# vsahni3/cross-attention-ViT

Hardware: AMD Instinct MI355X
Metric: 3D patch-tokens/sec fwd+bwd, 2-modality 128^3 p16 ViT (higher is better)
Workload: dtype bf16; 1 GPU; configs[1]: ModelCross d=768 H=12 mlp=3072 2x2 blocks, 2 modalities, 128^3 volume, 16^3 patches (N=513), dropout 0; per_gpu_batch=126, global_batch=126, seq_len=513, parallelism=dp1, step=zero-grad + weight bf16 cast + fwd + loss + bwd, optimizer_step=excluded, launch=eager (one launch per kernel)

## Files before the change

cross-attention-vit_amd/csrc/gemm.hip:

```cpp
#include "xvit_common.h"

#include <atomic>
#include <algorithm>
#include <string>

namespace xvit {

struct GemmParams {
  const bf16* A = nullptr; const bf16* B = nullptr; void* C = nullptr; const float* bias = nullptr; const float* res = nullptr; bf16* aux = nullptr;
  int64_t lda = 0, ldb = 0, ldc = 0, ldr = 0, ldaux = 0;
  int64_t sA = 0, sB = 0, sC = 0, sBias = 0, sR = 0, sAux = 0;
  int M = 0, N = 0, K = 0, k_per_split = 0, split_k = 1, ntm = 0, ntn = 0;
  int c_f32 = 0, act = XVIT_ACT_NONE, accumulate = 0;
  int res_row_mod = 0, res_row_off = 0, seg_rows = 0, seg_skip = 0, row_off = 0;
  float* slab = nullptr;
  float* colsum = nullptr;
  float drop_p = 0.f, drop_inv = 1.f; uint64_t drop_seed = 0;
  const uint64_t* drop_epoch = nullptr;
  int aux_deriv = 0;
  int narrow_epi = 0;
  int ncg = 1;
  int res_in_body = 0;
  struct PatchGather {
    int mode = 0;
// ... 508 lines not shown
template <int ACT, bool DROP, int R, bool PERM = false, bool RESPF = false>
__device__ __forceinline__ void big_epi_regions(const GemmParams& p, BigEpi& e, LoadCursor& lc, EpiLoads& cur, const f32x4 (&acc)[8][4], XVIT_LDS char* slice,
                                                const uint32_t (&woff)[8], const uint32_t (&roff)[4]) {
  if constexpr ((R & 3) == 0) {
#pragma unroll
    for (int i = 0; i < 4; ++i)
#pragma unroll
      for (int j = 0; j < 4; ++j) {
        if constexpr (PERM) *(XVIT_LDS f32x4*)(slice + (i >> 1) * 8192 + woff[(i & 1) * 4 + j]) = acc[(R >> 2) * 4 + i][j];
        else *(XVIT_LDS f32x4*)(slice + i * 4096 + woff[j]) = acc[(R >> 2) * 4 + i][j];
      }
  }
  EpiLoads nxt;
  if constexpr (ACT == XVIT_ACT_DGELU && R < 7) big_epi_issue_aux(p, e, lc, nxt);
  if constexpr (RESPF && R < 7) big_epi_issue_res(p, e, lc, nxt);
#pragma unroll
  for (int b = 0; b < 4; ++b) {
    const int it = (R & 3) * 4 + b;
    const f32x4 v = *(const XVIT_LDS f32x4*)(slice + it * 1024 + roff[it & 3]);
    big_epi_body<ACT, DROP, RESPF>(p, e, v, cur.aux[b], cur.res[b]);
  }
  __builtin_amdgcn_sched_barrier(0);
  if constexpr (R < 7) big_epi_regions<ACT, DROP, R + 1, PERM, RESPF>(p, e, lc, nxt, acc, slice, woff, roff);
}

template <int ACT, bool DROP, bool PERM = false, bool RESPF = false>
__device__ __forceinline__ void big_epilogue(const GemmParams& p, BigEpi& e, const f32x4 (&acc)[8][4], XVIT_LDS char* slice, const uint32_t (&woff)[8],
                                             const uint32_t (&roff)[4]) {
  LoadCursor lc = {e.row, e.aux, e.res, e.rrem};
  EpiLoads first;
  if constexpr (ACT == XVIT_ACT_DGELU) big_epi_issue_aux(p, e, lc, first);
  if constexpr (RESPF) big_epi_issue_res(p, e, lc, first);
  big_epi_regions<ACT, DROP, 0, PERM, RESPF>(p, e, lc, first, acc, slice, woff, roff);
  if (p.colsum && !e.to_slab) colsum_flush<16>(e.colsum_dst, e.csum, e.col_ok);
}

__device__ __forceinline__ int pin_lane(int lane) {
  int pin = 0;
  asm volatile("" : "+v"(pin));
  return lane + pin;
}

struct Transpose8 {
  uint32_t woff[4], roffw[2][2];
  __device__ __forceinline__ void init(int wl) {
    const int r = wl & 15, g = wl >> 4, c = wl & 7, rr = wl >> 3;
#pragma unroll
    for (int j = 0; j < 4; ++j) woff[j] = (uint32_t)(r * 256 + (((j * 4 + g) ^ r) << 4));
#pragma unroll
    for (int par = 0; par < 2; ++par)
#pragma unroll
      for (int k = 0; k < 2; ++k) roffw[par][k] = (uint32_t)(rr * 256 + (((2 * c + k) ^ ((par * 8 + rr) & 15)) << 4));
  }
  template <int PASS>
  __device__ __forceinline__ void write(XVIT_LDS char* slice, const f32x4 (&acc)[8][4]) const {
#pragma unroll
    for (int i = 0; i < 4; ++i)
#pragma unroll
      for (int j = 0; j < 4; ++j) *(XVIT_LDS f32x4*)(slice + i * 4096 + woff[j]) = acc[PASS * 4 + i][j];
  }
  __device__ __forceinline__ void read(const XVIT_LDS char* slice, int it, f32x4& v0, f32x4& v1) const {
    v0 = *(const XVIT_LDS f32x4*)(slice + it * 2048 + roffw[it & 1][0]);
    v1 = *(const XVIT_LDS f32x4*)(slice + it * 2048 + roffw[it & 1][1]);
  }
};
template <int R, class Loads, class Prefetch, class Body>
__device__ __forceinline__ void transpose8_regions(const Transpose8& t, const f32x4 (&acc)[8][4], XVIT_LDS char* slice, Loads& cur, const Prefetch& prefetch, const Body& body) {
  if constexpr ((R & 3) == 0) t.write<(R >> 2)>(slice, acc);
  Loads nxt;
  if constexpr (R < 7) prefetch(nxt);
#pragma unroll
  for (int b = 0; b < 2; ++b) {
    f32x4 v0, v1;
    t.read(slice, (R & 3) * 2 + b, v0, v1);
    body(v0, v1, cur, b);
  }
  __builtin_amdgcn_sched_barrier(0);
  if constexpr (R < 7) transpose8_regions<R + 1>(t, acc, slice, nxt, prefetch, body);
}

typedef __attribute__((ext_vector_type(8))) float f32x8;
struct WideEpi {
  __amdgpu_buffer_rsrc_t rc, raux;
  bool has_aux, col_ok;
  uint32_t col;
  f32x4 bias0, bias1, csum0, csum1;
  uint64_t drop_base;
  uint32_t row, c, aux, c_step, aux_step;
};
struct WideCursor { uint32_t row, aux; };
struct WideLoads { u32x4_t aux[2]; };

__device__ __forceinline__ void wide_issue_aux(const GemmParams& p, const WideEpi& e, WideCursor& lc, WideLoads& L) {
#pragma unroll
  for (int b = 0; b < 2; ++b) {
    const bool ok = e.col_ok && lc.row < (uint32_t)p.M;
    L.aux[b] = __builtin_amdgcn_raw_buffer_load_b128(e.raux, ok ? lc.aux : OOB, 0, XVIT_EPI_LOAD_AUX);
    lc.row += 8; lc.aux += e.aux_step;
  }
}

__device__ __forceinline__ u32x4_t pack_bf16x8(const f32x4& a, const f32x4& b) {
  return __builtin_bit_cast(u32x4_t, to_bf16x8(a, b));
}

template <int ACT, bool DROP>
__device__ __forceinline__ void wide_half(const GemmParams& p, f32x4& v, const bf16x4 z, uint64_t idx, u32x2_t& dpack) {
  f32x4 d;
  act4<ACT>(v, d, z);
  if (ACT == ACT_GELU_D) {
    dpack = __builtin_bit_cast(u32x2_t, to_bf16x4(d));
  }
  if (DROP) dropout4(p, v, idx);
}

template <int ACT, bool DROP>
__device__ __forceinline__ void wide_body(const GemmParams& p, WideEpi& e, f32x4 v0, f32x4 v1, u32x4_t auxv) {
  const bool ok = e.col_ok && e.row < (uint32_t)p.M;
  v0 += e.bias0; v1 += e.bias1;
  if (ACT == XVIT_ACT_GELU && e.has_aux) __builtin_amdgcn_raw_buffer_store_b128(pack_bf16x8(v0, v1), e.raux, ok ? e.aux : OOB, 0, XVIT_EPI_STORE_AUX);
  const bf16x8 z = __builtin_bit_cast(bf16x8, auxv);
  const uint64_t idx = e.drop_base + (uint64_t)e.row * p.N + e.col;
  u32x2_t d0 = {0u, 0u}, d1 = {0u, 0u};
  wide_half<ACT, DROP>(p, v0, bf16x4{z[0], z[1], z[2], z[3]}, idx, d0);
  if ((ACT != XVIT_ACT_NONE && ACT != ACT_MULAUX) || DROP) __builtin_amdgcn_sched_barrier(0);
  wide_half<ACT, DROP>(p, v1, bf16x4{z[4], z[5], z[6], z[7]}, idx + 4, d1);
  if (ACT == ACT_GELU_D && e.has_aux) __builtin_amdgcn_raw_buffer_store_b128(u32x4_t{d0[0], d0[1], d1[0], d1[1]}, e.raux, ok ? e.aux : OOB, 0, XVIT_EPI_STORE_AUX);
  __builtin_amdgcn_raw_buffer_store_b128(pack_bf16x8(v0, v1), e.rc, ok ? e.c : OOB, 0, XVIT_EPI_STORE_AUX);
#pragma unroll
  for (int c = 0; c < 4; ++c) { e.csum0[c] += ok ? v0[c] : 0.f; e.csum1[c] += ok ? v1[c] : 0.f; }
  e.row += 8; e.c += e.c_step; e.aux += e.aux_step;
}

template <int ACT, bool DROP>
__device__ __forceinline__ void wide_epilogue(const GemmParams& p, WideEpi& e, const f32x4 (&acc)[8][4], XVIT_LDS char* slice, const Transpose8& t, float* colsum_dst) {
  WideCursor lc = {e.row, e.aux};
  const auto prefetch = [&](WideLoads& L) {
    if constexpr (ACT == XVIT_ACT_DGELU || ACT == ACT_MULAUX) wide_issue_aux(p, e, lc, L);
  };
  WideLoads first;
  prefetch(first);
  transpose8_regions<0>(t, acc, slice, first, prefetch, [&](f32x4 v0, f32x4 v1, const WideLoads& cur, int b) { wide_body<ACT, DROP>(p, e, v0, v1, cur.aux[b]); });
  if (colsum_dst) {
    colsum_flush<8>(colsum_dst, e.csum0, e.col_ok);
    colsum_flush<8>(colsum_dst + 4, e.csum1, e.col_ok);
  }
}

template <int ACT>
__device__ __forceinline__ void wave_tile_epilogue_wide(const GemmParams& p, const f32x4 (&acc)[8][4], XVIT_LDS char* smem, int wave, int lane, int row0, int col0,
                                                        int batch) {
  WideEpi e;
  e.rc = make_rsrc((const char*)p.C + batch * p.sC * 2, clamp_bytes(0x7FFFFFF0ll));
  e.has_aux = p.aux != nullptr;
  const bool has_bias = p.bias != nullptr;
  e.raux = make_rsrc(e.has_aux ? (const void*)(p.aux + batch * p.sAux) : (const void*)p.C, e.has_aux ? 0x7FFFFFF0u : 0u);
  const __amdgpu_buffer_rsrc_t rbias = make_rsrc(has_bias ? (const void*)(p.bias + batch * p.sBias) : (const void*)p.C, has_bias ? (uint32_t)(p.N * 4) : 0u);
  const int wl = pin_lane(lane);
  Transpose8 t;
  t.init(wl);
  XVIT_LDS char* slice = smem + wave * EPI_WAVE_BYTES;
  e.col = (uint32_t)(col0 + (wl & 7) * 8);
  e.col_ok = e.col < (uint32_t)p.N;
  e.bias0 = __builtin_bit_cast(f32x4, __builtin_amdgcn_raw_buffer_load_b128(rbias, e.col * 4, 0, 0));
  e.bias1 = __builtin_bit_cast(f32x4, __builtin_amdgcn_raw_buffer_load_b128(rbias, e.col * 4 + 16, 0, 0));
  e.drop_base = (uint64_t)batch * ((uint64_t)p.M * p.N);
  e.csum0 = f32x4{0.f, 0.f, 0.f, 0.f}; e.csum1 = f32x4{0.f, 0.f, 0.f, 0.f};
  float* colsum_dst = p.colsum ? p.colsum + batch * p.sBias + e.col : nullptr;
  e.row = (uint32_t)(row0 + (wl >> 3));
  e.c = e.row * (uint32_t)p.ldc * 2u + e.col * 2u;
  e.aux = e.row * (uint32_t)p.ldaux * 2u + e.col * 2u;
  e.c_step = 8u * (uint32_t)p.ldc * 2u;
  e.aux_step = 8u * (uint32_t)p.ldaux * 2u;
  wide_epilogue<ACT, false>(p, e, acc, slice, t, colsum_dst);
}

template <bool PERM = false, bool RES_PF = true>
__device__ __forceinline__ void wave_tile_epilogue(const GemmParams& p, const f32x4 (&acc)[8][4], XVIT_LDS char* smem, int wave, int lane, int row0, int col0,
                                                   int batch, int split) {
  const int nbatch = gridDim.z / p.split_k;
  BigEpi e;
  const int64_t celt = p.c_f32 ? 4 : 2;
  e.rc = make_rsrc((const char*)p.C + batch * p.sC * celt, clamp_bytes(0x7FFFFFF0ll));
  e.has_aux = p.aux != nullptr; e.has_res = p.res != nullptr; e.to_slab = p.slab != nullptr;
  const bool has_bias = p.bias != nullptr;
  e.raux = make_rsrc(e.has_aux ? (const void*)(p.aux + batch * p.sAux) : (const void*)p.C, e.has_aux ? 0x7FFFFFF0u : 0u);
  e.rres = make_rsrc(e.has_res ? (const void*)(p.res + batch * p.sR) : (const void*)p.C, e.has_res ? 0x7FFFFFF0u : 0u);
  const __amdgpu_buffer_rsrc_t rbias = make_rsrc(has_bias ? (const void*)(p.bias + batch * p.sBias) : (const void*)p.C, has_bias ? (uint32_t)(p.N * 4) : 0u);
  e.rslab = make_rsrc(e.to_slab ? (const void*)(p.slab + ((int64_t)split * nbatch + batch) * (int64_t)p.M * p.N) : (const void*)p.C,
                      e.to_slab ? clamp_bytes((int64_t)p.M * p.N * 4) : 0u);
  const int wl = pin_lane(lane);
  uint32_t woff[8], roff[4];
  {
    const int r = wl & 15, g = wl >> 4, k = wl & 15, rr = wl >> 4;
#pragma unroll
    for (int j = 0; j < 4; ++j) woff[j] = woff[4 + j] = (uint32_t)(r * 256 + (((j * 4 + g) ^ r) << 4));
    if constexpr (PERM) {
#pragma unroll
      for (int half = 0; half < 2; ++half) {
        const int l32 = 16 * half + r, jj = l32 >> 3, ii = l32 & 7, rho = (ii & 3) * 8 + 2 * jj + (ii >> 2);
#pragma unroll
        for (int j = 0; j < 4; ++j) woff[half * 4 + j] = (uint32_t)(rho * 256 + (((j * 4 + g) ^ (rho & 15)) << 4));
      }
    }
#pragma unroll
    for (int q = 0; q < 4; ++q) roff[q] = (uint32_t)(rr * 256 + ((k ^ (q * 4 + rr)) << 4));
  }
  XVIT_LDS char* slice = smem + wave * EPI_WAVE_BYTES;
  e.col = (uint32_t)(col0 + (wl & 15) * 4);
  e.col_ok = e.col < (uint32_t)p.N;
  e.bias = __builtin_bit_cast(f32x4, __builtin_amdgcn_raw_buffer_load_b128(rbias, e.col * 4, 0, 0));
  e.drop_base = (uint64_t)batch * ((uint64_t)p.M * p.N);
  e.csum = f32x4{0.f, 0.f, 0.f, 0.f};
  e.colsum_dst = p.colsum ? p.colsum + batch * p.sBias + e.col : nullptr;
  e.row = (uint32_t)(row0 + (wl >> 4));
  {
    const bool rmap = p.res_row_mod > 0, smap = p.seg_rows > 0;
    e.rmod = rmap ? (uint32_t)p.res_row_mod : 0x7FFFFFFFu;
    e.smod = smap ? (uint32_t)p.seg_rows : 0x7FFFFFFFu;
    e.rrem = rmap ? e.row % e.rmod : e.row;
    e.srem = smap ? e.row % e.smod : e.row;
    const uint32_t rrow = rmap ? (uint32_t)p.res_row_off + e.rrem : e.row;
    const uint32_t orow = smap ? e.row + (e.row / e.smod) * (uint32_t)p.seg_skip + (uint32_t)p.row_off : e.row;
    const uint32_t ce = p.c_f32 ? 4u : 2u;
    e.c = orow * (uint32_t)p.ldc * ce + e.col * ce;
    e.aux = e.row * (uint32_t)p.ldaux * 2u + e.col * 2u;
    e.res = rrow * (uint32_t)p.ldr * 4u + e.col * 4u;
// ... 20 lines not shown
  if (p.drop_p > 0.f) {
    if (p.act == XVIT_ACT_GELU) big_epilogue<XVIT_ACT_GELU, true>(p, e, acc, slice, woff, roff);
    else if (p.act == XVIT_ACT_DGELU) big_epilogue<XVIT_ACT_DGELU, true>(p, e, acc, slice, woff, roff);
    else big_epilogue<XVIT_ACT_NONE, true>(p, e, acc, slice, woff, roff);
  } else if (p.act == XVIT_ACT_GELU) big_epilogue<XVIT_ACT_GELU, false>(p, e, acc, slice, woff, roff);
  else if (p.act == XVIT_ACT_DGELU) big_epilogue<XVIT_ACT_DGELU, false>(p, e, acc, slice, woff, roff);
  else big_epilogue<XVIT_ACT_NONE, false>(p, e, acc, slice, woff, roff);
}

struct ScatterEpi {
  char* vol;
  uint32_t eoff;
  bool col_ok;
  uint32_t row;
};

__device__ __forceinline__ void scatter_body(const GemmParams& p, ScatterEpi& e, f32x4 v0, f32x4 v1) {
  const GemmParams::PatchGather& g = p.g;
  const uint32_t row = e.row;
  e.row += 8;
  if (!e.col_ok || row >= (uint32_t)p.M) return;
  uint32_t n, b, d, w;
  const uint32_t smp = fast_div(row, (uint32_t)g.ntok, g.m_ntok, n);
  if (n < (uint32_t)g.cls) return;
  const uint32_t t = fast_div(n - (uint32_t)g.cls, (uint32_t)g.Dn, g.m_dn, d);
  const uint32_t h = fast_div(t, (uint32_t)g.Wn, g.m_wn, w);
  const uint32_t mod = fast_div(smp, (uint32_t)g.nb, g.m_nb, b);
  const uint32_t off = b * (uint32_t)g.sBt + mod * (uint32_t)g.sMd + d * (uint32_t)(g.dp * g.Sz) + h * (uint32_t)(g.hp * g.Sy) + w * (uint32_t)g.wp + e.eoff;
  if (p.c_f32) {
    f32x4* dst = (f32x4*)((float*)e.vol + off);
    dst[0] = v0;
    dst[1] = v1;
  } else {
    *(u32x4_t*)((bf16*)e.vol + off) = pack_bf16x8(v0, v1);
  }
}

__device__ __forceinline__ void scatter_epilogue(const GemmParams& p, const f32x4 (&acc)[8][4], XVIT_LDS char* smem, int wave, int lane, int row0, int col0) {
  const int wl = pin_lane(lane);
  Transpose8 t;
  t.init(wl);
  ScatterEpi e;
  e.vol = (char*)p.C;
  const uint32_t col = (uint32_t)(col0 + (wl & 7) * 8);
  e.col_ok = col < (uint32_t)p.N;
  e.eoff = e.col_ok ? gather_elem_off(p.g, (int)col) : 0u;
  e.row = (uint32_t)(row0 + (wl >> 3));
  struct NoLoads {} none;
  transpose8_regions<0>(t, acc, smem + wave * EPI_WAVE_BYTES, none, [](NoLoads&) {}, [&](f32x4 v0, f32x4 v1, const NoLoads&, int) { scatter_body(p, e, v0, v1); });
}

#ifdef XVIT_GEMM_CLOCK_PROBE
__device__ long long xvit_dbg_clk[2 * 4096];
struct ClockProbe {
  long long c0, w0;
  __device__ ClockProbe() : c0(clock64()), w0(wall_clock64()) {}
  __device__ ~ClockProbe() {
    if (threadIdx.x == 0 && blockIdx.z == 0 && blockIdx.x < 4096) { xvit_dbg_clk[2 * blockIdx.x] = clock64() - c0; xvit_dbg_clk[2 * blockIdx.x + 1] = wall_clock64() - w0; }
  }
};
#endif
template <bool A_KS, bool B_KS, int WIDE_ACT, int GATHER = 0>
__global__ __launch_bounds__(512, 2) void gemm_big_kernel(const GemmParams p) {
  extern __shared__ __attribute__((aligned(16))) char smem_raw[];
  XVIT_LDS char* smem = (XVIT_LDS char*)smem_raw;
#ifdef XVIT_GEMM_CLOCK_PROBE
  ClockProbe clock_probe;
#endif
  const int tid = threadIdx.x, lane = tid & 63, wave = uniform(tid >> 6);
  const int wr = wave >> 2, wc = wave & 3;

  const int nblk = gridDim.x;
  const int logical = xcd_logical(blockIdx.x + nblk * blockIdx.z, nblk * gridDim.z);
  const int zz = logical / nblk, tile = logical - zz * nblk;
  const int grp = min(tile / (p.ntm * p.ncg), (p.ntn - 1) / p.ncg);
  const int rem = tile - grp * p.ntm * p.ncg;
  const int gw = min(p.ncg, p.ntn - grp * p.ncg);
  const int tm = rem / gw, tn = grp * p.ncg + (rem - tm * gw);
  const int m0 = tm * TBM, n0 = tn * TBN;
  const int batch = zz / p.split_k, split = zz - batch * p.split_k;
  const int k_begin = split * p.k_per_split;
  const int k_end = min(p.K, k_begin + p.k_per_split);
  const int nk = (k_end - k_begin + BK - 1) / BK;

  TileLoader<A_KS, TBM> la;
  TileLoader<B_KS, TBN> lb;
  {
    const bf16* Ab = p.A + batch * p.sA;
    if constexpr (GATHER == 1) la.init_gather_rows(p.g, Ab, m0, p.M, wave, lane);
    else if constexpr (GATHER == 2 || GATHER == 3) {
      const int64_t rows = (int64_t)(p.K / p.g.pcount) * p.g.ntok;
      la.init(OperandTile{Ab + m0, ((rows - 1) * p.lda + (p.M - m0)) * 2}, p.lda, wave, lane, GATHER == 2 ? &p.g : nullptr);
    } else la.init(operand_tile<A_KS>(Ab, p.lda, m0, p.M, k_begin, k_end), p.lda, wave, lane);
    const bf16* Bb = p.B + batch * p.sB;
    if constexpr (GATHER == 2 || GATHER == 3) lb.init_gather_ks(p.g, Bb, n0, p.N, wave, lane);
    else lb.init(operand_tile<B_KS>(Bb, p.ldb, n0, p.N, k_begin, k_end), p.ldb, wave, lane);
  }
  const int ktg0 = k_begin / BK;
  uint32_t fix_a[4], fix_b[4];
  if constexpr (GATHER == 3) {
    la.init_token_fixed(p.g, m0, p.M, false, fix_a, wave, lane);
    lb.init_token_fixed(p.g, n0, p.N, true, fix_b, wave, lane);
  }
  auto step_off = [&](int kt, uint32_t& oa, uint32_t& ob) {
    if constexpr (GATHER == 1) { oa = gather_soff_rows(p.g, ktg0 + kt); ob = (uint32_t)kt * lb.kstep; }
    else if constexpr (GATHER == 2) { GatherStep o; o = gather_soff_wgrad(p.g, ktg0 + kt, p.lda); oa = o.a; ob = o.b; }
    else if constexpr (GATHER == 3) {
      la.place_tokens(p.g, ktg0 + kt, (uint32_t)p.K, p.lda, false, fix_a, wave, lane);
      lb.place_tokens(p.g, ktg0 + kt, (uint32_t)p.K, 0, true, fix_b, wave, lane);
      oa = ob = 0u;
    }
    else { oa = (uint32_t)kt * la.kstep; ob = (uint32_t)kt * lb.kstep; }
  };
  TileFrag<A_KS, TBM, 8> fa;
  TileFrag<B_KS, TBN, 4> fb;
  fa.init(wr * 8, lane);
  fb.init(wc * 4, lane);

  f32x4 acc[8][4];
#pragma unroll
  for (int i = 0; i < 8; ++i)
#pragma unroll
    for (int j = 0; j < 4; ++j) acc[i][j] = f32x4{0.f, 0.f, 0.f, 0.f};

  const __amdgpu_buffer_rsrc_t null_rsrc = make_rsrc(p.A, 0u);
  if (nk > 0) {
    uint32_t oa, ob;
    step_off(0, oa, ob);
    la.issue_at(smem, wave, oa);
    lb.issue_at(smem + T_OPER, wave, ob);
  }
  for (int kt = 0; kt < nk; ++kt) {
    asm volatile("s_waitcnt vmcnt(0)" ::: "memory");
    __syncthreads();
    const bool more = kt + 1 < nk;
    uint32_t soff_a, soff_b;
    step_off(kt + 1, soff_a, soff_b);
    XVIT_LDS char* nxt = smem + ((kt + 1) & 1) * T_STAGE;
    const XVIT_LDS char* sa = smem + (kt & 1) * T_STAGE;
    const XVIT_LDS char* sb = sa + T_OPER;
#ifndef XVIT_DEBUG_NO_MMA
    big_tile_mma<A_KS, B_KS>(sa, sb, fa, fb, acc, la, lb, more ? la.rsrc : null_rsrc, more ? lb.rsrc : null_rsrc, nxt, wave, soff_a, soff_b);
#endif
  }

  asm volatile("s_waitcnt vmcnt(0)" ::: "memory");
  __syncthreads();
  if constexpr (GATHER == 4) scatter_epilogue(p, acc, smem, wave, lane, m0 + wr * 128, n0 + wc * 64);
  else if constexpr (WIDE_ACT >= 0) wave_tile_epilogue_wide<WIDE_ACT>(p, acc, smem, wave, lane, m0 + wr * 128, n0 + wc * 64, batch);
  else wave_tile_epilogue<GATHER == 1, GATHER <= 1>(p, acc, smem, wave, lane, m0 + wr * 128, n0 + wc * 64, batch, split);
}

__global__ void splitk_epilogue_kernel(const GemmParams p, int nbatch) {
  const int nv = p.N >> 2;
  const int64_t per = (int64_t)p.M * nv, total = per * nbatch;
  for (int64_t i = (int64_t)blockIdx.x * blockDim.x + threadIdx.x; i < total; i += (int64_t)gridDim.x * blockDim.x) {
    const int b = (int)(i / per);
    const int64_t r = i - (int64_t)b * per;
    const int row = (int)(r / nv), col = (int)(r - (int64_t)row * nv) * 4;
    f32x4 v = {0.f, 0.f, 0.f, 0.f};
    for (int s = 0; s < p.split_k; ++s) v += *(const f32x4*)(p.slab + (((int64_t)s * nbatch + b) * p.M + row) * p.N + col);
    const f32x4 o = epilogue_apply_rt(p, v, row, col, b * p.sC, p.bias ? p.bias + b * p.sBias : nullptr, p.res ? p.res + b * p.sR : nullptr,
                                      p.aux ? p.aux + b * p.sAux : nullptr);
    if (p.colsum) {
#pragma unroll
      for (int e = 0; e < 4; ++e) unsafeAtomicAdd(p.colsum + b * p.sBias + col + e, o[e]);
    }
  }
}

}

using namespace xvit;

static bool aligned16(const void* p) { return (reinterpret_cast<uintptr_t>(p) & 15) == 0; }

static std::atomic<int> g_gemm_tile{0};
static std::atomic<int> g_gemm_epi{0};
static std::atomic<int> g_gemm_res_pf{0};
static std::atomic<int> g_gemm_group{0};

static bool use_big_tile(const xvit_gemm_args* a) {
  if (a->M < 256 || a->N < 256 || g_gemm_tile.load(std::memory_order_relaxed) == 1) return false;
  if (g_gemm_tile.load(std::memory_order_relaxed) == 2) return true;
  const int64_t big_blocks = (int64_t)((a->M + 255) / 256) * ((a->N + 255) / 256) * a->batch * (a->split_k > 0 ? a->split_k : 1);
  return big_blocks > 128;
}

static int k_per_split(int K, int split_k) {
  const int ktiles = (K + BK - 1) / BK;
  return ((ktiles + split_k - 1) / split_k) * BK;
}

static void set_tile_grid(GemmParams& p, int tile, int layout, bool grouped = true) {
  p.ntm = (p.M + tile - 1) / tile; p.ntn = (p.N + tile - 1) / tile;
  p.ncg = p.ntn;
  if (grouped) {
    const int forced = g_gemm_group.load(std::memory_order_relaxed);
    p.ncg = forced > 0 ? std::min(forced, p.ntn) : (layout == XVIT_GEMM_NT && p.ntn >= 6 ? 3 : p.ntn);
  }
}

template <bool A_KS, bool B_KS, int WIDE_ACT, int GATHER = 0>
static void launch_big(const GemmParams& p, int grid_z, hipStream_t s) {
  launch_lds<gemm_big_kernel<A_KS, B_KS, WIDE_ACT, GATHER>, T_LDS, 512>(dim3(p.ntm * p.ntn, 1, grid_z), s, p);
}
template <bool A_KS, bool B_KS>
static void launch_small(const GemmParams& p, int grid_z, hipStream_t s) {
  launch_lds<gemm_kernel<A_KS, B_KS>, GEMM_LDS, 256>(dim3(p.ntm * p.ntn, 1, grid_z), s, p);
}
static void launch_splitk_reduce(const GemmParams& p, int nbatch, hipStream_t s) {
  const int64_t work = (int64_t)nbatch * p.M * (p.N / 4);
  const int g = (int)((work + 255) / 256 > 4096 ? 4096 : (work + 255) / 256);
  hipLaunchKernelGGL(splitk_epilogue_kernel, dim3(g), dim3(256), 0, s, p, nbatch);
}

extern "C" int xvit_set_option(const char* name, int value) {
  XVIT_REQUIRE(name != nullptr, "xvit_set_option: null name");
  const std::string n(name);
  if (n == "gemm_tile") { XVIT_REQUIRE(value >= 0 && value <= 2, "xvit_set_option: gemm_tile must be 0 (auto), 1 (128x128 only) or 2 (256x256 whenever M, N >= 256)"); g_gemm_tile = value; return 0; }
  if (n == "gemm_group") { XVIT_REQUIRE(value >= 0 && value <= 4096, "xvit_set_option: gemm_group must be in [0, 4096]"); g_gemm_group = value; return 0; }
  if (n == "gemm_epilogue") { XVIT_REQUIRE(value == 0 || value == 1, "xvit_set_option: gemm_epilogue must be 0 (auto) or 1 (narrow)"); g_gemm_epi = value; return 0; }
  if (n == "gemm_res_prefetch") { XVIT_REQUIRE(value == 0 || value == 1, "xvit_set_option: gemm_res_prefetch must be 0 (one region ahead) or 1 (in the body)"); g_gemm_res_pf = value; return 0; }
  if (n == "attn_peel") { XVIT_REQUIRE(value >= 0 && value <= 2, "xvit_set_option: attn_peel must be 0 (token 0 stays on the tile grid), 1 (auto: large grids) or 2 (whenever N = 64 m + 1)"); set_attn_peel(value); return 0; }
  set_error("xvit_set_option: unknown option '%s'", name);
  return XVIT_ERR_ARG;
}

extern "C" int64_t xvit_gemm_workspace_bytes(const xvit_gemm_args* a) {
  if (!a || a->split_k <= 1) return 0;
  return (int64_t)a->split_k * a->batch * a->M * a->N * (int64_t)sizeof(float);
}

extern "C" int xvit_gemm(const xvit_gemm_args* a, xvit_stream_t stream) {
  XVIT_REQUIRE(a != nullptr, "xvit_gemm: null args");
  XVIT_REQUIRE(a->layout >= 0 && a->layout <= 2, "xvit_gemm: bad layout %d", a->layout);
  XVIT_REQUIRE(a->M > 0 && a->N > 0 && a->K > 0 && a->batch > 0, "xvit_gemm: M,N,K,batch must be > 0 (got %d,%d,%d,%d)", a->M, a->N, a->K, a->batch);
  XVIT_REQUIRE(a->A && a->B && a->C, "xvit_gemm: null A/B/C");
  const bool a_ks = a->layout == XVIT_GEMM_TN, b_ks = a->layout != XVIT_GEMM_NT;
  XVIT_REQUIRE(a_ks || a->K % 64 == 0, "xvit_gemm: K=%d must be a multiple of 64 when A is k-contiguous", a->K);
  XVIT_REQUIRE(b_ks || a->K % 64 == 0, "xvit_gemm: K=%d must be a multiple of 64 when B is k-contiguous", a->K);
  XVIT_REQUIRE(a->N % 4 == 0, "xvit_gemm: N=%d must be a multiple of 4 (use xvit_small_linear_*)", a->N);
  XVIT_REQUIRE(a->lda % 8 == 0 && a->ldb % 8 == 0 && a->stride_a % 8 == 0 && a->stride_b % 8 == 0, "xvit_gemm: lda/ldb/strides must be multiples of 8 elements");
  XVIT_REQUIRE(aligned16(a->A) && aligned16(a->B) && aligned16(a->C), "xvit_gemm: A/B/C must be 16-byte aligned");
  XVIT_REQUIRE(a->ldc % 4 == 0 && a->stride_c % 4 == 0, "xvit_gemm: ldc/stride_c must be multiples of 4");
  XVIT_REQUIRE(a->lda >= (a_ks ? a->M : a->K) && a->ldb >= (b_ks ? a->N : a->K) && a->ldc >= a->N, "xvit_gemm: leading dimension smaller than the row length");
  const int64_t a_rows = a_ks ? a->K : a->M, b_rows = b_ks ? a->K : a->N;
  XVIT_REQUIRE(a_rows * a->lda * 2 < (1ll << 31) && b_rows * a->ldb * 2 < (1ll << 31), "xvit_gemm: an operand matrix exceeds 2 GiB (unsupported addressing range)");
  XVIT_REQUIRE(a->split_k >= 1, "xvit_gemm: split_k must be >= 1");
  {
    const int64_t out_rows = a->out_seg_rows > 0 ? (int64_t)a->M + (a->M / a->out_seg_rows + 1) * a->out_seg_skip + a->out_row_off : a->M;
    XVIT_REQUIRE(out_rows * a->ldc * 4 < (1ll << 31) && (!a->aux || (int64_t)a->M * a->ldaux * 2 < (1ll << 31)) &&
                     (!a->residual || (int64_t)a->M * a->ldr * 4 < (1ll << 31)),
                 "xvit_gemm: C / aux / residual of one batch exceed 2 GiB (unsupported addressing range)");
  }
  XVIT_REQUIRE(!(a->accumulate && a->c_dtype != XVIT_F32), "xvit_gemm: accumulate needs fp32 C");
  XVIT_REQUIRE(a->act != XVIT_ACT_DGELU || a->aux, "xvit_gemm: ACT_DGELU needs aux (pre-activation)");
  XVIT_REQUIRE(a->aux_mode == 0 || a->aux_mode == 1, "xvit_gemm: aux_mode must be 0 (aux = pre-activation) or 1 (aux = GELU')");
  if (a->aux) XVIT_REQUIRE(a->ldaux % 4 == 0 && a->ldaux >= a->N && (reinterpret_cast<uintptr_t>(a->aux) & 7) == 0, "xvit_gemm: bad aux layout");
  if (a->residual) XVIT_REQUIRE(a->ldr % 4 == 0 && a->ldr >= a->N && aligned16(a->residual), "xvit_gemm: bad residual layout");
  if (a->bias) XVIT_REQUIRE(aligned16(a->bias) && a->stride_bias % 4 == 0, "xvit_gemm: bias must be 16-byte aligned");
  XVIT_REQUIRE((int64_t)a->batch * a->split_k <= 65535, "xvit_gemm: batch*split_k too large");
  const bool big = use_big_tile(a);
  const int64_t ws_need = xvit_gemm_workspace_bytes(a);
  if (ws_need > 0)
    XVIT_REQUIRE(a->workspace && a->workspace_bytes >= ws_need && aligned16(a->workspace), "xvit_gemm: split_k=%d needs %lld bytes of 16-byte aligned workspace (got %lld)",
                 a->split_k, (long long)ws_need, (long long)a->workspace_bytes);

  GemmParams p;
  p.A = (const bf16*)a->A; p.B = (const bf16*)a->B; p.C = a->C; p.bias = a->bias; p.res = a->residual; p.aux = (bf16*)a->aux;
  p.lda = a->lda; p.ldb = a->ldb; p.ldc = a->ldc; p.ldr = a->ldr; p.ldaux = a->ldaux;
  p.sA = a->stride_a; p.sB = a->stride_b; p.sC = a->stride_c; p.sBias = a->stride_bias; p.sR = a->stride_r; p.sAux = a->stride_aux;
  p.M = a->M; p.N = a->N; p.K = a->K; p.split_k = a->split_k;
  p.k_per_split = k_per_split(a->K, a->split_k);
  p.c_f32 = a->c_dtype == XVIT_F32; p.act = a->act; p.accumulate = a->accumulate;
  p.res_row_mod = a->res_row_mod; p.res_row_off = a->res_row_off;
  p.seg_rows = a->out_seg_rows; p.seg_skip = a->out_seg_skip; p.row_off = a->out_row_off;
  p.slab = ws_need > 0 ? (float*)a->workspace : nullptr;
  p.colsum = a->colsum;
  XVIT_REQUIRE(a->dropout_p >= 0.f && a->dropout_p < 1.f, "xvit_gemm: dropout_p must be in [0, 1)");
  p.drop_p = a->dropout_p; p.drop_inv = 1.0f / (1.0f - a->dropout_p); p.drop_seed = a->dropout_seed;
  p.drop_epoch = a->dropout_p > 0.f ? drop_epoch_ptr() : nullptr;
  p.narrow_epi = g_gemm_epi.load(std::memory_order_relaxed);
  p.res_in_body = g_gemm_res_pf.load(std::memory_order_relaxed);
  p.aux_deriv = a->aux_mode;
  hipStream_t s = (hipStream_t)stream;
  const int gz = a->batch * a->split_k;

  if (big) {
    set_tile_grid(p, TBM, a->layout);
    const bool wide = !p.c_f32 && !p.slab && !p.res && p.seg_rows == 0 && !p.narrow_epi && p.drop_p == 0.f && a->layout != XVIT_GEMM_TN &&
                      ((p.N | (int)p.ldc | (int)p.ldaux) & 7) == 0 && (a->layout == XVIT_GEMM_NT ? p.act != XVIT_ACT_DGELU : p.act != XVIT_ACT_GELU);
    if (wide && a->layout == XVIT_GEMM_NT && p.act == XVIT_ACT_NONE) launch_big<false, false, XVIT_ACT_NONE>(p, gz, s);
    else if (wide && a->layout == XVIT_GEMM_NT && p.aux_deriv) launch_big<false, false, ACT_GELU_D>(p, gz, s);
    else if (wide && a->layout == XVIT_GEMM_NT) launch_big<false, false, XVIT_ACT_GELU>(p, gz, s);
    else if (wide && p.act == XVIT_ACT_NONE) launch_big<false, true, XVIT_ACT_NONE>(p, gz, s);
    else if (wide && p.aux_deriv) launch_big<false, true, ACT_MULAUX>(p, gz, s);
    else if (wide) launch_big<false, true, XVIT_ACT_DGELU>(p, gz, s);
    else if (a->layout == XVIT_GEMM_NT) launch_big<false, false, -1>(p, gz, s);
    else if (a->layout == XVIT_GEMM_NN) launch_big<false, true, -1>(p, gz, s);
    else launch_big<true, true, -1>(p, gz, s);
  } else {
    set_tile_grid(p, BM, a->layout, false);
    switch (a->layout) {
      case XVIT_GEMM_NT: launch_small<false, false>(p, gz, s); break;
      case XVIT_GEMM_NN: launch_small<false, true>(p, gz, s); break;
      default: launch_small<true, true>(p, gz, s); break;
    }
  }
  if (p.slab) launch_splitk_reduce(p, a->batch, s);
  return check_launch("xvit_gemm");
}

static int64_t pe_rows(const xvit_patch_geom* g) {
  return (int64_t)g->M * g->B * (g->cls_rows + (int64_t)(g->D / g->dp) * (g->H / g->hp) * (g->W / g->wp));
}

static bool pe_geom_ok(const xvit_patch_geom* g) {
  if (!g || g->B <= 0 || g->M <= 0 || g->dp <= 0 || g->hp <= 0 || g->wp <= 0 || (g->cls_rows != 0 && g->cls_rows != 1)) return false;
  return !(g->D % g->dp || g->H % g->hp || g->W % g->wp);
}

extern "C" int xvit_patch_embed_supported(const xvit_patch_geom* g, int d) {
  if (!pe_geom_ok(g)) return 0;
  const int Dn = g->D / g->dp, Hn = g->H / g->hp, Wn = g->W / g->wp;
  const int64_t pd = (int64_t)g->dp * g->hp * g->wp, pcount = (int64_t)Dn * Hn * Wn;
  if (g->wp % 8 || 64 % g->wp || (g->hp * g->wp) % 64) return 0;
  if (pd % 256 || d % 256 || d < 256) return 0;
  const int64_t rows = pe_rows(g);
  if (rows < 2048) return 0;
  if ((int64_t)g->B * g->M * g->D * g->H * g->W * 2 >= (1ll << 31)) return 0;
  if (rows * d * 4 >= (1ll << 31) || pcount > (1 << 24)) return 0;
  return 1;
}

static bool pe_aligned(const xvit_patch_geom* g) {
  const int Dn = g->D / g->dp, Wn = g->W / g->wp;
  return 64 % Dn == 0 && (Dn * Wn) % 64 == 0;
}

static void pe_fill(GemmParams& p, const xvit_patch_geom* g, int mode) {
  p.g.mode = mode;
  p.g.dp = g->dp; p.g.hp = g->hp; p.g.wp = g->wp;
  p.g.Dn = g->D / g->dp; p.g.Wn = g->W / g->wp;
  p.g.Sy = g->W; p.g.Sz = g->H * g->W;
  p.g.pcount = (g->D / g->dp) * (g->H / g->hp) * (g->W / g->wp);
  p.g.cls = g->cls_rows; p.g.ntok = p.g.cls + p.g.pcount;
  p.g.nb = g->B;
  p.g.sMd = (int64_t)g->D * g->H * g->W; p.g.sBt = p.g.sMd * g->M;
  p.g.vol_bytes = (uint32_t)((int64_t)g->B * g->M * g->D * g->H * g->W * 2);
  auto magic = [](int d) { return d <= 1 ? 0xFFFFFFFFu : (uint32_t)((1ull << 32) / (uint64_t)d); };
// ... 57 lines not shown
  const bool aligned = pe_aligned(g);
  pe_fill(p, g, aligned ? 2 : 3);
  p.A = (const bf16*)dx; p.B = (const bf16*)img; p.C = dW;
  p.lda = lddx; p.ldc = lddw;
  p.M = d; p.N = (int)pd;
  p.K = (int)((int64_t)g->M * g->B * p.g.pcount);
  p.split_k = pe_wgrad_split(g, d);
  p.k_per_split = k_per_split(p.K, p.split_k);
  p.slab = need > 0 ? (float*)workspace : nullptr;
  set_tile_grid(p, TBM, XVIT_GEMM_TN, false);
  hipStream_t s = (hipStream_t)stream;
  if (aligned) launch_big<true, true, -1, 2>(p, p.split_k, s);
  else launch_big<true, true, -1, 3>(p, p.split_k, s);
  if (p.slab) launch_splitk_reduce(p, 1, s);
  return check_launch("xvit_patch_embed_wgrad");
}

extern "C" int xvit_patch_embed_dgrad_supported(const xvit_patch_geom* g, int d) {
  if (!pe_geom_ok(g)) return 0;
  if (g->wp % 8) return 0;
  if (d % 64 || d < 64) return 0;
  const int64_t rows = pe_rows(g);
  if (rows < 2048) return 0;
  if ((int64_t)g->B * g->M * g->D * g->H * g->W >= (1ll << 30)) return 0;
  if (rows * d * 2 >= (1ll << 31)) return 0;
  if ((int64_t)(g->D / g->dp) * (g->H / g->hp) * (g->W / g->wp) > (1 << 24)) return 0;
  return 1;
}

extern "C" int xvit_patch_embed_dgrad(const void* dx, int64_t lddx, const void* W, int64_t ldw, const xvit_patch_geom* g, int d, void* dimg, int dimg_dtype,
                                      xvit_stream_t stream) {
  XVIT_REQUIRE(dx && W && g && dimg, "xvit_patch_embed_dgrad: null pointer");
  XVIT_REQUIRE(dimg_dtype == XVIT_F32 || dimg_dtype == XVIT_BF16, "xvit_patch_embed_dgrad: bad output dtype %d", dimg_dtype);
  XVIT_REQUIRE(xvit_patch_embed_dgrad_supported(g, d) == 1, "xvit_patch_embed_dgrad: geometry not supported by the fused kernel (xvit_patch_embed_dgrad_supported)");
  const int64_t pd = (int64_t)g->dp * g->hp * g->wp;
  XVIT_REQUIRE(lddx >= d && lddx % 8 == 0 && ldw >= pd && ldw % 8 == 0, "xvit_patch_embed_dgrad: bad leading dimension");
  XVIT_REQUIRE(aligned16(dx) && aligned16(W) && aligned16(dimg), "xvit_patch_embed_dgrad: pointers must be 16-byte aligned");
  XVIT_REQUIRE(pe_rows(g) * lddx * 2 < (1ll << 31) && (int64_t)d * ldw * 2 < (1ll << 31), "xvit_patch_embed_dgrad: an operand exceeds 2 GiB (unsupported addressing range)");
  GemmParams p;
  pe_defaults(p);
  pe_fill(p, g, 4);
  p.A = (const bf16*)dx; p.B = (const bf16*)W; p.C = dimg;
  p.lda = lddx; p.ldb = ldw;
  p.M = (int)pe_rows(g); p.N = (int)pd; p.K = d;
  p.k_per_split = p.K;
  p.c_f32 = dimg_dtype == XVIT_F32;
  set_tile_grid(p, TBM, XVIT_GEMM_NN);
  launch_big<false, true, -1, 4>(p, 1, (hipStream_t)stream);
  return check_launch("xvit_patch_embed_dgrad");
}

#ifdef XVIT_GEMM_CLOCK_PROBE
extern "C" int xvit_dbg_read_clk(long long* out, int n) { return (int)hipMemcpyFromSymbol(out, HIP_SYMBOL(xvit::xvit_dbg_clk), (size_t)n * 16); }
#endif
```

Measured before the change: 3.785 million patch-tokens/s.

## Add persistent tile-loop GEMM kernel overlapping next tile loads with epilogue

```diff
diff --git a/cross-attention-vit_amd/csrc/gemm.hip b/cross-attention-vit_amd/csrc/gemm.hip
--- a/cross-attention-vit_amd/csrc/gemm.hip
+++ b/cross-attention-vit_amd/csrc/gemm.hip
@@ -584,31 +584,32 @@
 #pragma unroll
       for (int k = 0; k < 2; ++k) roffw[par][k] = (uint32_t)(rr * 256 + (((2 * c + k) ^ ((par * 8 + rr) & 15)) << 4));
   }
-  template <int PASS>
+  template <int FIRST, int COUNT>
   __device__ __forceinline__ void write(XVIT_LDS char* slice, const f32x4 (&acc)[8][4]) const {
 #pragma unroll
-    for (int i = 0; i < 4; ++i)
-#pragma unroll
-      for (int j = 0; j < 4; ++j) *(XVIT_LDS f32x4*)(slice + i * 4096 + woff[j]) = acc[PASS * 4 + i][j];
+    for (int i = 0; i < COUNT; ++i)
+#pragma unroll
+      for (int j = 0; j < 4; ++j) *(XVIT_LDS f32x4*)(slice + i * 4096 + woff[j]) = acc[FIRST + i][j];
   }
   __device__ __forceinline__ void read(const XVIT_LDS char* slice, int it, f32x4& v0, f32x4& v1) const {
     v0 = *(const XVIT_LDS f32x4*)(slice + it * 2048 + roffw[it & 1][0]);
     v1 = *(const XVIT_LDS f32x4*)(slice + it * 2048 + roffw[it & 1][1]);
   }
 };
-template <int R, class Loads, class Prefetch, class Body>
+template <int R, int PASS = 64, class Loads, class Prefetch, class Body>
 __device__ __forceinline__ void transpose8_regions(const Transpose8& t, const f32x4 (&acc)[8][4], XVIT_LDS char* slice, Loads& cur, const Prefetch& prefetch, const Body& body) {
-  if constexpr ((R & 3) == 0) t.write<(R >> 2)>(slice, acc);
+  constexpr int RPP = PASS / 16;
+  if constexpr (R % RPP == 0) t.write<R, RPP>(slice, acc);
   Loads nxt;
   if constexpr (R < 7) prefetch(nxt);
 #pragma unroll
   for (int b = 0; b < 2; ++b) {
     f32x4 v0, v1;
-    t.read(slice, (R & 3) * 2 + b, v0, v1);
+    t.read(slice, (R % RPP) * 2 + b, v0, v1);
     body(v0, v1, cur, b);
   }
   __builtin_amdgcn_sched_barrier(0);
-  if constexpr (R < 7) transpose8_regions<R + 1>(t, acc, slice, nxt, prefetch, body);
+  if constexpr (R < 7) transpose8_regions<R + 1, PASS>(t, acc, slice, nxt, prefetch, body);
 }
 
 typedef __attribute__((ext_vector_type(8))) float f32x8;
@@ -664,7 +665,7 @@
   e.row += 8; e.c += e.c_step; e.aux += e.aux_step;
 }
 
-template <int ACT, bool DROP>
+template <int ACT, bool DROP, int PASS = 64>
 __device__ __forceinline__ void wide_epilogue(const GemmParams& p, WideEpi& e, const f32x4 (&acc)[8][4], XVIT_LDS char* slice, const Transpose8& t, float* colsum_dst) {
   WideCursor lc = {e.row, e.aux};
   const auto prefetch = [&](WideLoads& L) {
@@ -672,14 +673,14 @@
   };
   WideLoads first;
   prefetch(first);
-  transpose8_regions<0>(t, acc, slice, first, prefetch, [&](f32x4 v0, f32x4 v1, const WideLoads& cur, int b) { wide_body<ACT, DROP>(p, e, v0, v1, cur.aux[b]); });
+  transpose8_regions<0, PASS>(t, acc, slice, first, prefetch, [&](f32x4 v0, f32x4 v1, const WideLoads& cur, int b) { wide_body<ACT, DROP>(p, e, v0, v1, cur.aux[b]); });
   if (colsum_dst) {
     colsum_flush<8>(colsum_dst, e.csum0, e.col_ok);
     colsum_flush<8>(colsum_dst + 4, e.csum1, e.col_ok);
   }
 }
 
-template <int ACT>
+template <int ACT, int PASS = 64>
 __device__ __forceinline__ void wave_tile_epilogue_wide(const GemmParams& p, const f32x4 (&acc)[8][4], XVIT_LDS char* smem, int wave, int lane, int row0, int col0,
                                                         int batch) {
   WideEpi e;
@@ -691,7 +692,7 @@
   const int wl = pin_lane(lane);
   Transpose8 t;
   t.init(wl);
-  XVIT_LDS char* slice = smem + wave * EPI_WAVE_BYTES;
+  XVIT_LDS char* slice = smem + wave * (PASS * 256);
   e.col = (uint32_t)(col0 + (wl & 7) * 8);
   e.col_ok = e.col < (uint32_t)p.N;
   e.bias0 = __builtin_bit_cast(f32x4, __builtin_amdgcn_raw_buffer_load_b128(rbias, e.col * 4, 0, 0));
@@ -704,7 +705,7 @@
   e.aux = e.row * (uint32_t)p.ldaux * 2u + e.col * 2u;
   e.c_step = 8u * (uint32_t)p.ldc * 2u;
   e.aux_step = 8u * (uint32_t)p.ldaux * 2u;
-  wide_epilogue<ACT, false>(p, e, acc, slice, t, colsum_dst);
+  wide_epilogue<ACT, false, PASS>(p, e, acc, slice, t, colsum_dst);
 }
 
 template <bool PERM = false, bool RES_PF = true>
@@ -831,13 +832,21 @@
 
 #ifdef XVIT_GEMM_CLOCK_PROBE
 __device__ long long xvit_dbg_clk[2 * 4096];
+__device__ long long xvit_dbg_seg[3 * 4096];
 struct ClockProbe {
-  long long c0, w0;
+  long long c0, w0, t[3] = {0, 0, 0};
   __device__ ClockProbe() : c0(clock64()), w0(wall_clock64()) {}
+  __device__ void mark(int i) { if (t[i] == 0) t[i] = clock64(); }
   __device__ ~ClockProbe() {
-    if (threadIdx.x == 0 && blockIdx.z == 0 && blockIdx.x < 4096) { xvit_dbg_clk[2 * blockIdx.x] = clock64() - c0; xvit_dbg_clk[2 * blockIdx.x + 1] = wall_clock64() - w0; }
+    if (threadIdx.x == 0 && blockIdx.z == 0 && blockIdx.x < 4096) {
+      xvit_dbg_clk[2 * blockIdx.x] = clock64() - c0; xvit_dbg_clk[2 * blockIdx.x + 1] = wall_clock64() - w0;
+      for (int i = 0; i < 3; ++i) xvit_dbg_seg[3 * blockIdx.x + i] = t[i] - c0;
+    }
   }
 };
+#define XVIT_PROBE_MARK(i) clock_probe.mark(i)
+#else
+#define XVIT_PROBE_MARK(i)
 #endif
 template <bool A_KS, bool B_KS, int WIDE_ACT, int GATHER = 0>
 __global__ __launch_bounds__(512, 2) void gemm_big_kernel(const GemmParams p) {
@@ -912,6 +921,7 @@
   for (int kt = 0; kt < nk; ++kt) {
     asm volatile("s_waitcnt vmcnt(0)" ::: "memory");
     __syncthreads();
+    XVIT_PROBE_MARK(0);
     const bool more = kt + 1 < nk;
     uint32_t soff_a, soff_b;
     step_off(kt + 1, soff_a, soff_b);
@@ -922,12 +932,114 @@
     big_tile_mma<A_KS, B_KS>(sa, sb, fa, fb, acc, la, lb, more ? la.rsrc : null_rsrc, more ? lb.rsrc : null_rsrc, nxt, wave, soff_a, soff_b);
 #endif
   }
+  XVIT_PROBE_MARK(1);
 
   asm volatile("s_waitcnt vmcnt(0)" ::: "memory");
   __syncthreads();
   if constexpr (GATHER == 4) scatter_epilogue(p, acc, smem, wave, lane, m0 + wr * 128, n0 + wc * 64);
   else if constexpr (WIDE_ACT >= 0) wave_tile_epilogue_wide<WIDE_ACT>(p, acc, smem, wave, lane, m0 + wr * 128, n0 + wc * 64, batch);
   else wave_tile_epilogue<GATHER == 1, GATHER <= 1>(p, acc, smem, wave, lane, m0 + wr * 128, n0 + wc * 64, batch, split);
+  XVIT_PROBE_MARK(2);
+}
+
+__device__ __forceinline__ const GemmParams& reload_params() {
+  auto q = __builtin_amdgcn_kernarg_segment_ptr();
+  asm volatile("" : "+s"(q));
+  return *(const GemmParams*)q;
+}
+
+template <bool B_KS, int WIDE_ACT>
+__global__ __launch_bounds__(512, 2) void gemm_big_loop_kernel(const GemmParams p) {
+  extern __shared__ __attribute__((aligned(16))) char smem_raw[];
+  XVIT_LDS char* smem = (XVIT_LDS char*)smem_raw;
+#ifdef XVIT_GEMM_CLOCK_PROBE
+  ClockProbe clock_probe;
+#endif
+  static_assert(WIDE_ACT >= 0, "the tile loop exists behind the wide epilogues only");
+  constexpr int EPI_STORES = 16;
+  const int tid = threadIdx.x, lane = tid & 63, wave = uniform(tid >> 6);
+  const int wr = wave >> 2, wc = wave & 3;
+  auto tile_origin = [](const GemmParams& q, int slot, int& m0, int& n0) {
+    const int tile = xcd_logical(slot, q.ntm * q.ntn);
+    const int grp = min(tile / (q.ntm * q.ncg), (q.ntn - 1) / q.ncg);
+    const int rem = tile - grp * q.ntm * q.ncg;
+    const int gw = min(q.ncg, q.ntn - grp * q.ncg);
+    const int tm = rem / gw, tn = grp * q.ncg + (rem - tm * gw);
+    m0 = tm * TBM; n0 = tn * TBN;
+  };
+  auto tile_rsrc = [](const GemmParams& q, int m0, int n0, __amdgpu_buffer_rsrc_t& ra, __amdgpu_buffer_rsrc_t& rb) {
+    const OperandTile ta = operand_tile<false>(q.A, q.lda, m0, q.M, 0, q.K), tb = operand_tile<B_KS>(q.B, q.ldb, n0, q.N, 0, q.K);
+    ra = make_rsrc(ta.base, clamp_bytes(ta.bytes));
+    rb = make_rsrc(tb.base, clamp_bytes(tb.bytes));
+  };
+  TileLoader<false, TBM> la;
+  TileLoader<B_KS, TBN> lb;
+  la.init(OperandTile{p.A, 0}, p.lda, wave, lane);
+  lb.init(OperandTile{p.B, 0}, p.ldb, wave, lane);
+  TileFrag<false, TBM, 8> fa;
+  TileFrag<B_KS, TBN, 4> fb;
+  fa.init(wr * 8, lane);
+  fb.init(wc * 4, lane);
+
+  int slot = blockIdx.x;
+  int stage = 0;
+  int m0, n0;
+  tile_origin(p, slot, m0, n0);
+  tile_rsrc(p, m0, n0, la.rsrc, lb.rsrc);
+  la.issue_at(smem, wave, 0u);
+  lb.issue_at(smem + T_OPER, wave, 0u);
+  for (;;) {
+    const bool first = slot == (int)blockIdx.x;
+    const int nk = (reload_params().K + BK - 1) / BK;
+    f32x4 acc[8][4];
+#pragma unroll
+    for (int i = 0; i < 8; ++i)
+#pragma unroll
+      for (int j = 0; j < 4; ++j) acc[i][j] = f32x4{0.f, 0.f, 0.f, 0.f};
+    for (int kt = 0; kt + 1 < nk; ++kt) {
+      if (kt == 0 && !first) wait_vmcnt<EPI_STORES>();
+      else wait_vmcnt<0>();
+      __syncthreads();
+      XVIT_PROBE_MARK(0);
+      XVIT_LDS char* nxt = smem + ((stage + kt + 1) & 1) * T_STAGE;
+      const XVIT_LDS char* sa = smem + ((stage + kt) & 1) * T_STAGE;
+      big_tile_mma<false, B_KS>(sa, sa + T_OPER, fa, fb, acc, la, lb, la.rsrc, lb.rsrc, nxt, wave, (uint32_t)(kt + 1) * la.kstep, (uint32_t)(kt + 1) * lb.kstep);
+    }
+    bool more;
+    int nm0 = 0, nn0 = 0;
+    __amdgpu_buffer_rsrc_t ra = make_rsrc(nullptr, 0u), rb = ra;
+    {
+      const GemmParams& q = reload_params();
+      more = slot + (int)gridDim.x < q.ntm * q.ntn;
+      if (more) {
+        tile_origin(q, slot + (int)gridDim.x, nm0, nn0);
+        tile_rsrc(q, nm0, nn0, ra, rb);
+      }
+    }
+    if (nk == 1 && !first) wait_vmcnt<EPI_STORES>();
+    else wait_vmcnt<0>();
+    __syncthreads();
+    XVIT_PROBE_MARK(0);
+    {
+      const XVIT_LDS char* sa = smem + ((stage + nk - 1) & 1) * T_STAGE;
+      big_tile_mma<false, B_KS>(sa, sa + T_OPER, fa, fb, acc, la, lb, ra, rb, smem + ((stage + nk) & 1) * T_STAGE, wave, 0u, 0u);
+    }
+    XVIT_PROBE_MARK(1);
+    if (!more) wait_vmcnt<0>();
+    __syncthreads();
+    {
+      const GemmParams& q = reload_params();
+      const int te = pin_lane(tid), we = uniform(te >> 6);
+      XVIT_LDS char* slices = smem + ((stage + nk - 1) & 1) * T_STAGE;
+      wave_tile_epilogue_wide<WIDE_ACT, 32>(q, acc, slices, we, te & 63, m0 + (we >> 2) * 128, n0 + (we & 3) * 64, 0);
+    }
+    XVIT_PROBE_MARK(2);
+    if (!more) break;
+    la.rsrc = ra; lb.rsrc = rb;
+    m0 = nm0; n0 = nn0;
+    slot += (int)gridDim.x;
+    stage = (stage + nk) & 1;
+  }
 }
 
 __global__ void splitk_epilogue_kernel(const GemmParams p, int nbatch) {
@@ -959,6 +1071,28 @@
 static std::atomic<int> g_gemm_res_pf{0};
 static std::atomic<int> g_gemm_group{0};
 
+static std::atomic<int> g_gemm_persist{0};
+
+static int cu_count() {
+  static const int n = [] {
+    int dev = 0, v = 0;
+    if (hipGetDevice(&dev) != hipSuccess || hipDeviceGetAttribute(&v, hipDeviceAttributeMultiprocessorCount, dev) != hipSuccess) v = 0;
+    return v;
+  }();
+  return n;
+}
+
+static int loop_workgroups(const xvit_gemm_args* a, const GemmParams& p, int grid_z) {
+  const int opt = g_gemm_persist.load(std::memory_order_relaxed);
+  if (opt == 1 || a->layout == XVIT_GEMM_TN || grid_z != 1) return 0;
+  const int tiles = p.ntm * p.ntn;
+  if (opt >= 2) return std::min(tiles, opt);
+  const int cus = cu_count();
+  if (cus <= 0 || tiles < 2 * cus) return 0;
+  if (p.K > 768 || (p.act != XVIT_ACT_NONE && !p.aux_deriv)) return 0;
+  return cus;
+}
+
 static bool use_big_tile(const xvit_gemm_args* a) {
   if (a->M < 256 || a->N < 256 || g_gemm_tile.load(std::memory_order_relaxed) == 1) return false;
   if (g_gemm_tile.load(std::memory_order_relaxed) == 2) return true;
@@ -984,6 +1118,10 @@
 static void launch_big(const GemmParams& p, int grid_z, hipStream_t s) {
   launch_lds<gemm_big_kernel<A_KS, B_KS, WIDE_ACT, GATHER>, T_LDS, 512>(dim3(p.ntm * p.ntn, 1, grid_z), s, p);
 }
+template <bool B_KS, int WIDE_ACT>
+static void launch_loop(const GemmParams& p, int wgs, hipStream_t s) {
+  launch_lds<gemm_big_loop_kernel<B_KS, WIDE_ACT>, T_LDS, 512>(dim3(wgs, 1, 1), s, p);
+}
 template <bool A_KS, bool B_KS>
 static void launch_small(const GemmParams& p, int grid_z, hipStream_t s) {
   launch_lds<gemm_kernel<A_KS, B_KS>, GEMM_LDS, 256>(dim3(p.ntm * p.ntn, 1, grid_z), s, p);
@@ -1000,6 +1138,7 @@
   if (n == "gemm_tile") { XVIT_REQUIRE(value >= 0 && value <= 2, "xvit_set_option: gemm_tile must be 0 (auto), 1 (128x128 only) or 2 (256x256 whenever M, N >= 256)"); g_gemm_tile = value; return 0; }
   if (n == "gemm_group") { XVIT_REQUIRE(value >= 0 && value <= 4096, "xvit_set_option: gemm_group must be in [0, 4096]"); g_gemm_group = value; return 0; }
   if (n == "gemm_epilogue") { XVIT_REQUIRE(value == 0 || value == 1, "xvit_set_option: gemm_epilogue must be 0 (auto) or 1 (narrow)"); g_gemm_epi = value; return 0; }
+  if (n == "gemm_persistent") { XVIT_REQUIRE(value >= 0 && value <= 4096, "xvit_set_option: gemm_persistent must be 0 (auto), 1 (one workgroup per tile) or 2..4096 (the tile loop on at most that many workgroups)"); g_gemm_persist = value; return 0; }
   if (n == "gemm_res_prefetch") { XVIT_REQUIRE(value == 0 || value == 1, "xvit_set_option: gemm_res_prefetch must be 0 (one region ahead) or 1 (in the body)"); g_gemm_res_pf = value; return 0; }
   if (n == "attn_peel") { XVIT_REQUIRE(value >= 0 && value <= 2, "xvit_set_option: attn_peel must be 0 (token 0 stays on the tile grid), 1 (auto: large grids) or 2 (whenever N = 64 m + 1)"); set_attn_peel(value); return 0; }
   set_error("xvit_set_option: unknown option '%s'", name);
@@ -1070,12 +1209,13 @@
     set_tile_grid(p, TBM, a->layout);
     const bool wide = !p.c_f32 && !p.slab && !p.res && p.seg_rows == 0 && !p.narrow_epi && p.drop_p == 0.f && a->layout != XVIT_GEMM_TN &&
                       ((p.N | (int)p.ldc | (int)p.ldaux) & 7) == 0 && (a->layout == XVIT_GEMM_NT ? p.act != XVIT_ACT_DGELU : p.act != XVIT_ACT_GELU);
-    if (wide && a->layout == XVIT_GEMM_NT && p.act == XVIT_ACT_NONE) launch_big<false, false, XVIT_ACT_NONE>(p, gz, s);
-    else if (wide && a->layout == XVIT_GEMM_NT && p.aux_deriv) launch_big<false, false, ACT_GELU_D>(p, gz, s);
-    else if (wide && a->layout == XVIT_GEMM_NT) launch_big<false, false, XVIT_ACT_GELU>(p, gz, s);
-    else if (wide && p.act == XVIT_ACT_NONE) launch_big<false, true, XVIT_ACT_NONE>(p, gz, s);
-    else if (wide && p.aux_deriv) launch_big<false, true, ACT_MULAUX>(p, gz, s);
-    else if (wide) launch_big<false, true, XVIT_ACT_DGELU>(p, gz, s);
+    const int lw = wide ? loop_workgroups(a, p, gz) : 0;
+    if (wide && a->layout == XVIT_GEMM_NT && p.act == XVIT_ACT_NONE) lw ? launch_loop<false, XVIT_ACT_NONE>(p, lw, s) : launch_big<false, false, XVIT_ACT_NONE>(p, gz, s);
+    else if (wide && a->layout == XVIT_GEMM_NT && p.aux_deriv) lw ? launch_loop<false, ACT_GELU_D>(p, lw, s) : launch_big<false, false, ACT_GELU_D>(p, gz, s);
+    else if (wide && a->layout == XVIT_GEMM_NT) lw ? launch_loop<false, XVIT_ACT_GELU>(p, lw, s) : launch_big<false, false, XVIT_ACT_GELU>(p, gz, s);
+    else if (wide && p.act == XVIT_ACT_NONE) lw ? launch_loop<true, XVIT_ACT_NONE>(p, lw, s) : launch_big<false, true, XVIT_ACT_NONE>(p, gz, s);
+    else if (wide && p.aux_deriv) lw ? launch_loop<true, ACT_MULAUX>(p, lw, s) : launch_big<false, true, ACT_MULAUX>(p, gz, s);
+    else if (wide) lw ? launch_loop<true, XVIT_ACT_DGELU>(p, lw, s) : launch_big<false, true, XVIT_ACT_DGELU>(p, gz, s);
     else if (a->layout == XVIT_GEMM_NT) launch_big<false, false, -1>(p, gz, s);
     else if (a->layout == XVIT_GEMM_NN) launch_big<false, true, -1>(p, gz, s);
     else launch_big<true, true, -1>(p, gz, s);
@@ -1239,4 +1379,5 @@
 
 #ifdef XVIT_GEMM_CLOCK_PROBE
 extern "C" int xvit_dbg_read_clk(long long* out, int n) { return (int)hipMemcpyFromSymbol(out, HIP_SYMBOL(xvit::xvit_dbg_clk), (size_t)n * 16); }
+extern "C" int xvit_dbg_read_seg(long long* out, int n) { return (int)hipMemcpyFromSymbol(out, HIP_SYMBOL(xvit::xvit_dbg_seg), (size_t)n * 24); }
 #endif
```

Measured after the change: 3.833 million patch-tokens/s, median of 6. 1.3% higher.
